# zzengcs/kubeML

Measured on AMD Instinct MI355X. Metric: images/sec (whole node) + epoch time, ResNet-34 CIFAR-10 at 1/2/4/8 workers, higher is better.
Workload: dtype bf16; 1 GPU; model=resnet34 (torchvision, ImageNet stem, 1000-class head), global_batch=256, per_worker_batch=256, image=32x32x3, parallelism=dp1, optimizer=SGD lr=0.01 wd=1e-4, sync=none (N=1: no collective in the step), graph=True, overlap_segments=False, graph_comm=False, grad_comm_dtype=fp32, sgd_rider=4f:321;123:s, step=kubeml_amd.engine.dp.make_train_step

## Files before the change

csrc/kernels/conv_igemm.hip:

```cpp
#include "kml_common.h"
#include "kml_sgd.h"

#include <type_traits>

namespace {

constexpr int PADK = 16;
constexpr int PADR = 8;

enum { FWD = 0, DGRAD = 1, WGRAD = 2 };

struct FastDiv {
  unsigned m;
  int s;
  int d;
};
__device__ __forceinline__ int fdiv(int n, const FastDiv& f) {
  return (int)(((unsigned long long)(unsigned)n * f.m) >> f.s);
}

struct ConvArgs {
  const bf16_t* x;
  const bf16_t* w;
  const bf16_t* dy;
// ... 1622 lines not shown
      return *reinterpret_cast<const bf16x8_t*>(base + (row * CPR + (c ^ (row & 15))) * 16);
    };
    f32x4_t acc[MR][NR];
#pragma unroll
    for (int i = 0; i < MR; ++i)
#pragma unroll
      for (int j = 0; j < NR; ++j) acc[i][j] = f32x4_t{0.f, 0.f, 0.f, 0.f};
    constexpr int KS = KD / 32;
    bf16x8_t af[2][MR], bf[2][NR];
#pragma unroll
    for (int i = 0; i < MR; ++i) af[0][i] = rd(sA, wm * WM + i * 16 + (lane & 15), 0);
#pragma unroll
    for (int j = 0; j < NR; ++j) bf[0][j] = rd(sB, wn * WN + j * 16 + (lane & 15), 0);
#pragma unroll
    for (int ks = 0; ks < KS; ++ks) {
      if (ks + 1 < KS) {
#pragma unroll
        for (int i = 0; i < MR; ++i) af[(ks + 1) & 1][i] = rd(sA, wm * WM + i * 16 + (lane & 15), ks + 1);
#pragma unroll
        for (int j = 0; j < NR; ++j) bf[(ks + 1) & 1][j] = rd(sB, wn * WN + j * 16 + (lane & 15), ks + 1);
      }
#pragma unroll
      for (int i = 0; i < MR; ++i)
#pragma unroll
        for (int j = 0; j < NR; ++j)
          acc[i][j] = __builtin_amdgcn_mfma_f32_16x16x32_bf16(af[ks & 1][i], bf[ks & 1][j], acc[i][j], 0, 0, 0);
    }
    __syncthreads();
    conv_epilogue<FWD, MR, NR, WM, WN, false, true>(a, acc, m0, n0, wm, wn, lane, tid, 0, 0,
                                                    reinterpret_cast<unsigned*>(smem));
  }
};

template <int MODE, int BM, int BN, int KD>
struct OneShotBwdBody {
  static_assert(MODE == DGRAD || MODE == WGRAD, "one-shot backward: dgrad / wgrad");
  static constexpr bool A_KC = MODE == DGRAD;
  static constexpr int A_BYTES = BM * KD * 2, B_BYTES = BN * KD * 2;
  static constexpr int WM = BM / 2, WN = BN / 2, MR = WM / 16, NR = WN / 16;
  static constexpr int NIA = A_BYTES / 1024, NIB = B_BYTES / 1024;
  static constexpr int SMEM_EPI = 16 + BM * (BN + 8) * 2 + 2 * BN * 4;
  static constexpr int SMEM = A_BYTES + B_BYTES > SMEM_EPI ? A_BYTES + B_BYTES : SMEM_EPI;
  static constexpr int THREADS = 256;
  static_assert(NIA % 4 == 0 && NIB % 4 == 0 && (KD / 8) % 16 == 0, "one-shot panel shape");
  static_assert((BM == 32 || BM == 64) && (BN == 32 || BN == 64), "K-strided tiles of 32 / 64 columns");
  static_assert(SMEM <= 160 * 1024, "one-shot panels exceed LDS");

  template <int R>
  __device__ __forceinline__ static void ks_slot(int L, int& k, int& lc) {
    k = L / (R / 8);
    lc = (L % (R / 8)) ^ swz_ks<R>(k);
  }

  __device__ __forceinline__ static void run(const ConvArgs& a, const Blk& bk, char* smem) {
    const int tid = threadIdx.x, lane = tid & 63, wave = tid >> 6, wm = wave >> 1, wn = wave & 1;
    const int m0 = bk.y * BM, n0 = bk.x * BN;
    const int tapoff = (a.r0 * a.KW + a.s0) * a.C;
    char* const sA = smem;
    char* const sB = smem + A_BYTES;
#pragma unroll
    for (int j = 0; j < NIA / 4; ++j) {
      const int u = j * 4 + wave, L = u * 64 + lane;
      const bf16_t* src;
      if constexpr (MODE == DGRAD) {
        const int row = L / (KD / 8), lc = (L % (KD / 8)) ^ (row & 15), m = m0 + row;
        src = m < a.M ? a.dy + (long long)m * a.K + lc * 8 : a.zp;
      } else {
        int k, lc;
        ks_slot<BM>(L, k, lc);
        const int col = m0 + lc * 8;
        src = (k < a.Kd && col < a.M) ? a.dy + (long long)k * a.K + col : a.zp;
      }
      __builtin_amdgcn_global_load_lds((const void*)src, (__attribute__((address_space(3))) void*)(sA + u * 1024),
                                       16, 0, 0);
    }
#pragma unroll
    for (int j = 0; j < NIB / 4; ++j) {
      const int u = j * 4 + wave, L = u * 64 + lane;
      int k, lc;
      ks_slot<BN>(L, k, lc);
      const int col = n0 + lc * 8;
      const bf16_t* src = a.zp;
      if constexpr (MODE == DGRAD) {
        if (k < a.K && col < a.N) {
          if (a.g22) {
            const int p = fdiv(k, a.fd_gK), q = fdiv(col, a.fd_gC);
            src = a.w + ((long long)(k - p * a.fd_gK.d) * 9 + tap22(p, q)) * a.fd_gC.d + (col - q * a.fd_gC.d);
          } else {
            src = a.w + (long long)k * a.KH * a.KW * a.C + tapoff + col;
          }
        }
      } else {
        if (k < a.Kd && col < a.N) src = a.x + (long long)k * a.C + col;
      }
      __builtin_amdgcn_global_load_lds((const void*)src, (__attribute__((address_space(3))) void*)(sB + u * 1024),
                                       16, 0, 0);
    }
    asm volatile("s_waitcnt vmcnt(0)" ::: "memory");
    __syncthreads();
    auto rdA = [&](int i, int ks) -> bf16x8_t {
      if constexpr (A_KC) {
        const int row = wm * WM + i * 16 + (lane & 15), c = 4 * ks + (lane >> 4);
        return *reinterpret_cast<const bf16x8_t*>(sA + (row * (KD / 8) + (c ^ (row & 15))) * 16);
      } else {
        return frag_kstrided<BM>(reinterpret_cast<const bf16_t*>(sA), wm * WM + i * 16, ks, lane);
      }
    };
    auto rdB = [&](int j, int ks) -> bf16x8_t {
      return frag_kstrided<BN>(reinterpret_cast<const bf16_t*>(sB), wn * WN + j * 16, ks, lane);
    };
    f32x4_t acc[MR][NR];
#pragma unroll
    for (int i = 0; i < MR; ++i)
#pragma unroll
      for (int j = 0; j < NR; ++j) acc[i][j] = f32x4_t{0.f, 0.f, 0.f, 0.f};
    constexpr int KS = KD / 32;
    bf16x8_t af[2][MR], bf[2][NR];
#pragma unroll
    for (int i = 0; i < MR; ++i) af[0][i] = rdA(i, 0);
#pragma unroll
    for (int j = 0; j < NR; ++j) bf[0][j] = rdB(j, 0);
#pragma unroll
    for (int ks = 0; ks < KS; ++ks) {
      if (ks + 1 < KS) {
#pragma unroll
        for (int i = 0; i < MR; ++i) af[(ks + 1) & 1][i] = rdA(i, ks + 1);
#pragma unroll
        for (int j = 0; j < NR; ++j) bf[(ks + 1) & 1][j] = rdB(j, ks + 1);
      }
#pragma unroll
      for (int i = 0; i < MR; ++i)
#pragma unroll
        for (int j = 0; j < NR; ++j)
          acc[i][j] = __builtin_amdgcn_mfma_f32_16x16x32_bf16(af[ks & 1][i], bf[ks & 1][j], acc[i][j], 0, 0, 0);
    }
    __syncthreads();
    conv_epilogue<MODE, MR, NR, WM, WN, false, true>(a, acc, m0, n0, wm, wn, lane, tid, 0, 0,
                                                     reinterpret_cast<unsigned*>(smem));
  }
};

template <int MODE, int BM, int BN, int KD>
__global__ __launch_bounds__(256) void k_conv_oneshot_bwd(ConvArgs a) {
  using Body = OneShotBwdBody<MODE, BM, BN, KD>;
  __shared__ __attribute__((aligned(1024))) char smem[Body::SMEM];
  Body::run(a, xcd_blk(), smem);
}

template <int MODE>
int dispatch_oneshot_bwd(const ConvArgs& a, int bm, int bn, hipStream_t s) {
  dim3 grid((a.N + bn - 1) / bn, (a.M + bm - 1) / bm, 1);
#define KML_OB(BMv, BNv, KDv)                                                              \
  if (bm == BMv && bn == BNv && a.Kd == KDv) {                                             \
    hipLaunchKernelGGL((k_conv_oneshot_bwd<MODE, BMv, BNv, KDv>), grid, dim3(256), 0, s, a); \
    KML_LAUNCH_CHECK();                                                                    \
  }
  if constexpr (MODE == DGRAD) {
    KML_OB(32, 32, 1024) KML_OB(32, 32, 512) KML_OB(32, 64, 512)
  } else {
    KML_OB(32, 32, 256) KML_OB(64, 32, 256) KML_OB(32, 64, 256) KML_OB(64, 64, 256)
  }
#undef KML_OB
  return (int)hipErrorInvalidValue;
}

template <int BM, int BN, int KD>
__global__ __launch_bounds__(256) void k_conv_oneshot(ConvArgs a) {
  using Body = OneShotBody<BM, BN, KD>;
  __shared__ __attribute__((aligned(1024))) char smem[Body::SMEM];
  Body::run(a, xcd_blk(), smem);
}
// ... 311 lines not shown
  if (id >= nd + nw) {
    kml_sgd_rider_run(rider, id - nd - nw);
    return;
  }
  if (id < nd) {
    Blk b;
    b.gx = dgx;
    b.x = id % dgx;
    const int t = id / dgx;
    b.y = t % dgy;
    b.z = t / dgy;
    DB::run(ad, b, smem);
  } else {
    id -= nd;
    Blk b;
    b.gx = wgx;
    b.x = id % wgx;
    const int t = id / wgx;
    b.y = t % wgy;
    b.z = t / wgy;
    WB::run(aw, b, smem);
  }
}

using DgIg3264 = IgemmBody<DGRAD, 32, 64, 64, true>;
using DgIg3232 = IgemmBody<DGRAD, 32, 32, 64, true>;
using DgDi3232 = DirectBody<DGRAD, 2, 2, 4, 4>;
using DgDi3216 = DirectBody<DGRAD, 2, 1, 4, 4>;
using DgDi6432 = DirectBody<DGRAD, 4, 2, 4, 2>;
using WgIg3232 = IgemmBody<WGRAD, 32, 32, 64, true>;
using WgIg6432 = IgemmBody<WGRAD, 64, 32, 64, true>;
using DgHa64x8 = HaloBody<DGRAD, 64, 8, 1, 32, 1>;
using DgHa128x4 = HaloBody<DGRAD, 128, 4, 4, 32, 1>;
#define KML_PAIR_LIST(X)                                   \
  X(4, 64, 32, 1032, DgHa64x8, 64, 32, WgIg3232, 32, 32)   \
  X(4, 64, 32, 1032, DgHa64x8, 64, 32, WgIg6432, 64, 32)   \
  X(4, 64, 32, 2052, DgHa128x4, 64, 32, WgIg3232, 32, 32)  \
  X(4, 64, 32, 2052, DgHa128x4, 64, 32, WgIg6432, 64, 32)  \
  X(0, 32, 64, 64, DgIg3264, 32, 64, WgIg3232, 32, 32)     \
  X(0, 32, 64, 64, DgIg3264, 32, 64, WgIg6432, 64, 32)     \
  X(0, 32, 32, 64, DgIg3232, 32, 32, WgIg3232, 32, 32)     \
  X(0, 32, 32, 64, DgIg3232, 32, 32, WgIg6432, 64, 32)     \
  X(3, 32, 32, 4, DgDi3232, 32, 32, WgIg3232, 32, 32)      \
  X(3, 32, 32, 4, DgDi3232, 32, 32, WgIg6432, 64, 32)      \
  X(3, 32, 16, 4, DgDi3216, 32, 16, WgIg3232, 32, 32)      \
  X(3, 32, 16, 4, DgDi3216, 32, 16, WgIg6432, 64, 32)      \
  X(3, 64, 32, 4, DgDi6432, 64, 32, WgIg3232, 32, 32)      \
  X(3, 64, 32, 4, DgDi6432, 64, 32, WgIg6432, 64, 32)

template <class DB, class WB>
int launch_pair(const ConvArgs& ad, int dbm, int dbn, const ConvArgs& aw, int wbm, int wbn, hipStream_t s) {
  const int dgx = (ad.N + dbn - 1) / dbn, dgy = (ad.M + dbm - 1) / dbm;
  const int wgx = (aw.N + wbn - 1) / wbn, wgy = (aw.M + wbm - 1) / wbm;
  const long long nd = (long long)dgx * dgy * ad.splits, nw = (long long)wgx * wgy * aw.splits;
  const KmlSgdRider rider = kml_rider_take();
  if (nd + nw + rider.blocks > 0x7fffffffLL) return (int)hipErrorInvalidValue;
  hipLaunchKernelGGL((k_conv_pair<DB, WB>), dim3((unsigned)(nd + nw + rider.blocks)), dim3(256), 0, s, ad, aw, dgx,
                     dgy, wgx, wgy, (int)nd, (int)nw, rider);
  KML_LAUNCH_CHECK();
}

int pair_index(int dv, int dbm, int dbn, int dbk, int wv, int wbm, int wbn, int wbk) {
  int idx = 0;
#define KML_PAIR_FIND(DV, DBM, DBN, DBK, DB, DTM, DTN, WB, WBM, WBN)                                   \
  ++idx;                                                                                             \
  if (dv == DV && dbm == DBM && dbn == DBN && dbk == DBK && wv == 0 && wbm == WBM && wbn == WBN && wbk == 64) \
    return idx;
  KML_PAIR_LIST(KML_PAIR_FIND)
#undef KML_PAIR_FIND
  return 0;
}

int dispatch_pair(int which, const ConvArgs& ad, const ConvArgs& aw, hipStream_t s) {
  int idx = 0;
#define KML_PAIR_RUN(DV, DBM, DBN, DBK, DB, DTM, DTN, WB, WBM, WBN) \
  if (++idx == which) return launch_pair<DB, WB>(ad, DTM, DTN, aw, WBM, WBN, s);
  KML_PAIR_LIST(KML_PAIR_RUN)
#undef KML_PAIR_RUN
  return (int)hipErrorInvalidValue;
}

template <class B1, class B2>
__global__ __launch_bounds__(256) void k_conv_fwd_pair(ConvArgs a1, ConvArgs a2, int g1x, int g1y, int g2x, int n1,
                                                       int n2) {
  static_assert(B1::THREADS == 256 && B2::THREADS == 256, "paired bodies run 256-thread blocks");
  constexpr int SM = B1::SMEM > B2::SMEM ? B1::SMEM : B2::SMEM;
  __shared__ __attribute__((aligned(1024))) char smem[SM];
  const int nwg = n1 + n2, lin = (int)blockIdx.x;
  const int q = nwg >> 3, r = nwg & 7, x = lin & 7, k = lin >> 3;
  int id = (x < r ? x * (q + 1) : r * (q + 1) + (x - r) * q) + k;
  Blk b;
  if (id < n1) {
    b.gx = g1x;
    b.x = id % g1x;
    b.y = id / g1x;
    b.z = 0;
    (void)g1y;
    B1::run(a1, b, smem);
  } else {
    id -= n1;
    b.gx = g2x;
    b.x = id % g2x;
    b.y = id / g2x;
    b.z = 0;
    B2::run(a2, b, smem);
  }
}

// ... 338 lines not shown
  set_splits(a, bk, splits);
  if (a.splits > 1 && (!slab || !counters)) return (int)hipErrorInvalidValue;
  a.slab = slab; a.counters = counters;
  a.accumulate = accumulate ? 1 : 0;
  return 0;
}
}

KML_API int kml_conv_pair_supported(int dvariant, int dbm, int dbn, int dbk, int wvariant, int wbm, int wbn, int wbk) {
  return pair_index(dvariant, dbm, dbn, dbk, wvariant, wbm, wbn, wbk) > 0 ? 1 : 0;
}

KML_API int kml_conv_bwd_pair(const bf16_t* dy, const bf16_t* w, const bf16_t* wt, bf16_t* dx, const bf16_t* addend,
                              const bf16_t* bnf_y, const bf16_t* bnf_c, const float* bnf_mean, const float* bnf_rstd,
                              float* bnf_part, float* grp_out, unsigned* grp_cnt, int grp_tiles, const bf16_t* x,
                              float* dw, int B, int H, int W, int C, int K, int KH,
                              int KW, int sh, int sw, int ph, int pw, int dbm, int dbn, int dbk, int dsplits,
                              int dvariant, float* slab, unsigned* counters, int wbm, int wbn, int wbk, int wsplits,
                              int wvariant, int fold_c, int bnf_mask_out, float* wslab, unsigned* wcounters,
                              int waccumulate, float* wbias, int wbias_acc, int g22, hipStream_t s) {
  const int which = pair_index(dvariant, dbm, dbn, dbk, wvariant, wbm, wbn, wbk);
  if (!which) return (int)hipErrorInvalidValue;
  if (dvariant == 4 && (g22 || fold_c || dsplits != 1 || dbk != K * 16 + H ||
                        !halo_shape_ok(H, W, K, C, KH, KW, sh, sw, ph, pw, dbm, dbn)))
    return (int)hipErrorInvalidValue;
  ConvArgs ad, aw;
  int e = prep_dgrad(ad, dy, w, wt, dx, addend, bnf_y, bnf_c, bnf_mean, bnf_rstd, bnf_part, grp_out, grp_cnt,
                     grp_tiles, B, H, W, C, K, KH, KW, sh, sw, ph, pw, dbk, dsplits, dvariant, slab, counters,
                     fold_c, bnf_mask_out, g22);
  if (e) return e;
  e = prep_wgrad(aw, x, dy, dw, B, H, W, C, K, KH, KW, sh, sw, ph, pw, wbk, wsplits, wvariant, waccumulate, wslab,
                 wcounters, wbias, wbias_acc);
  if (e) return e;
  return dispatch_pair(which, ad, aw, s);
}

KML_API int kml_weight_transpose_multi(const bf16_t* const* ws, bf16_t* const* wts, const int* dims, int n,
                                       hipStream_t s) {
  if (n < 1 || n > 16) return (int)hipErrorInvalidValue;
  TransposeBatch tb = {};
  tb.n = n;
  long long tiles = 0;
  for (int i = 0; i < n; ++i) {
    TransposeJob& j = tb.j[i];
    j.w = ws[i]; j.wt = wts[i];
    j.K = dims[4 * i]; j.T = dims[4 * i + 1]; j.C = dims[4 * i + 2];
    if (j.C % 8) return (int)hipErrorInvalidValue;
    j.Kp = (j.K + 31) / 32 * 32;
    j.tk = (j.Kp + 63) / 64;
    j.tc = (j.C + 63) / 64;
    j.tile_begin = (int)tiles;
    tiles += (long long)j.T * j.tk * j.tc;
  }
  if (tiles <= 0 || tiles > 0x7fffffffLL) return (int)hipErrorInvalidValue;
  hipLaunchKernelGGL(k_weight_transpose_multi, dim3((unsigned)tiles), dim3(256), 0, s, tb);
  KML_LAUNCH_CHECK();
}

KML_API int kml_conv_unroll22_multi(const bf16_t* const* ws, bf16_t* const* wus, const int* dims, int n,
                                    hipStream_t s) {
  if (n < 1 || n > 16) return (int)hipErrorInvalidValue;
  UnrollBatch ub = {};
  ub.n = n;
  long long blocks = 0;
  for (int i = 0; i < n; ++i) {
    UnrollJob& j = ub.j[i];
// ... 194 lines not shown
```

kubeml_amd/nn/fused.py:

```python
from __future__ import annotations

from typing import List, Optional

import torch
from torch.autograd import Function

import os

from .flat import grad_out, grad_out_pair, master_of, shadow_of

_BN_FUSE = True


def _wg_buf(conv, x):
    Kc, _, _, C = conv.weight._kml_grad_storage.shape
    shape = (4 * Kc, 1, 1, 4 * C)
    buf = getattr(conv, "_kml_wg_buf", None)
    if buf is None or tuple(buf.shape) != shape or buf.device != x.device:
        buf = torch.empty(shape, dtype=torch.float32, device=x.device)
        object.__setattr__(conv, "_kml_wg_buf", buf)
    return buf


def _wgrad_target(conv, x, unroll):
# ... 187 lines not shown
        c = K.conv_fwd(x, w, kh, kw, conv.stride, conv.padding, bias=bias)
        y = K.bn_apply(c, None, gamma, beta, res=res, run_mean=bn.running_mean, run_var=bn.running_var,
                       eps=bn.eps, relu=relu, training=False)
        return y, None

    @staticmethod
    def backward(dy, saved, conv, bn, want_dres: bool, need_dx: bool, addend=None, partial=None, consumer=None):
        dc, dres, wu = ConvBNUnit.bn_backward(dy, saved, conv, bn, want_dres, partial)
        dx, part_out = ConvBNUnit.conv_backward(dc, saved, conv, need_dx, wu, addend, consumer)
        return dx, dres, part_out

    @staticmethod
    def bn_backward(dy, saved, conv, bn, want_dres: bool, partial=None):
        from ..ops import kernels as K
        x, c, y, mean, rstd = saved
        dg, db, acc = grad_out_pair(bn.weight, bn.bias)
        wu = getattr(conv, "_kml_wu", None) if x.is_cuda else None
        dres = torch.empty_like(dy) if want_dres else None
        dc = K.bn_bwd(dy, None if partial is not None else y, c, mean, rstd, master_of(bn.weight),
                      dg, db, dres=dres, partial=partial, accumulate=acc, rider=_take_rider(bn))
        object.__setattr__(conv, "_kml_wu", None)
        return dc, dres, wu

    @staticmethod
    def conv_backward(dc, saved, conv, need_dx: bool, wu, addend=None, consumer=None):
        from ..ops import kernels as K
        x = saved[0]
        kh, kw = conv.kernel_size
        dx, part_out = None, None
        bnf = None if consumer is None else (consumer[2], consumer[1], consumer[3], consumer[4])
        if need_dx:
            w = shadow_of(conv.weight)
            wt = getattr(conv, "_kml_wt", None)
            if wt is None and K.bwd_plans(x.shape, w.shape[0], kh, kw, conv.stride, conv.padding,
                                          unroll=wu is not None)[0][4] == K.DIRECT:
                object.__setattr__(conv, "_kml_wants_wt", True)
            dw, acc = _wgrad_target(conv, x, wu is not None)
            r = K.conv_bwd(dc, w, x, dw, kh, kw, conv.stride, conv.padding,
                           addend=addend, bnf=bnf, wt=wt, wu=wu, bnf_mask=True, accumulate=acc,
                           rider=_take_rider(conv))
            if wu is not None:
                conv.weight._kml_flat.defer_fold22(conv.weight, dw)
            object.__setattr__(conv, "_kml_wt", None)
            dx, part_out = r if bnf is not None else (r, None)
            return dx, part_out
        _wgrad(x, dc, conv, unroll=wu is not None, rider=_take_rider(conv))
        if need_dx:
            r = K.conv_dgrad(dc, shadow_of(conv.weight), x.shape, kh, kw, conv.stride, conv.padding,
                             addend=addend, bnf=bnf, wu=wu, bnf_mask=True)
            dx, part_out = r if bnf is not None else (r, None)
        return dx, part_out


def _take_rider(conv):
    r = getattr(conv, "_kml_rider", None)
    return r() if r is not None else None


class PendingBN:
    __slots__ = ("y", "c", "rows", "G", "bn", "res", "mean", "rstd", "relu")

    def __init__(self, y, c, rows, G, bn, res, mean, rstd, relu):
        self.y, self.c, self.rows, self.G, self.bn = y, c, rows, G, bn
        self.res, self.mean, self.rstd, self.relu = res, mean, rstd, relu

    def materialize(self):
        from ..ops import kernels as K
        bn = self.bn
        K.bn_apply(self.c, self.rows, master_of(bn.weight), master_of(bn.bias), y=self.y, res=self.res,
                   save_mean=self.mean, save_rstd=self.rstd, run_mean=bn.running_mean, run_var=bn.running_var,
                   eps=bn.eps, momentum=bn.momentum if bn.momentum is not None else 0.1, relu=self.relu,
                   stats_rows=self.G)


# ... 233 lines not shown
```

kubeml_amd/ops/kernels.py:

```python
from __future__ import annotations

import contextlib
import json
import math
import os

import torch

from .. import _native
from .._native import HIP

BF16 = torch.bfloat16
F32 = torch.float32


def _s() -> int:
    return _native.stream_ptr()


def _p(t) -> int:
    return 0 if t is None else t.data_ptr()


def _chk(t, dtype, name, ndim=None):
# ... 432 lines not shown
def gemm_dgrad_gather_ok(C, K, stride) -> bool:
    return tuple(stride) == (1, 1) and K % 64 == 0 and C % 8 == 0


def gemm_conv_ok(C, K, H, W, KH, KW, stride, pad) -> bool:
    return C % 64 == 0 and K % 8 == 0


def oneshot_ok(C, K, Kd, H, W, KH, KW, stride, pad, bm, bn) -> bool:
    if Kd != C or (bm, bn) not in _ONESHOT_TILES.get(Kd, ()):
        return False
    r0, r1, s0, s1 = tap_window(H, W, KH, KW, stride[0], stride[1], pad[0], pad[1])
    OH, OW = out_hw(H, W, KH, KW, stride[0], stride[1], pad[0], pad[1])
    rows = (H * W == 1 and OH * OW == 1) or ((KH, KW) == (1, 1) and tuple(stride) == (1, 1) and tuple(pad) == (0, 0))
    return (r1 - r0) == 1 and (s1 - s0) == 1 and rows


_ONESHOT_MAX_ROWS = 4096


def oneshot_plan(C, K, Kd, H, W, KH, KW, stride, pad, B=0):
    if B * H * W > _ONESHOT_MAX_ROWS:
        return None
    for bm, bn in _ONESHOT_TILES.get(Kd, ()):
        if oneshot_ok(C, K, Kd, H, W, KH, KW, stride, pad, bm, bn):
            return (bm, bn, 0, 1, ONESHOT)
    return None


_ONESHOT_BWD_ON = False
_ONESHOT_DG_TILES = {1024: (32, 32), 512: (32, 32)}
_ONESHOT_WG_TILES = {256: (32, 32)}


def oneshot_bwd_plans(C, K, B, H, W, KH, KW, stride, pad):
    if not _ONESHOT_BWD_ON or C % 32 or K % 32:
        return None, None
    r0, r1, s0, s1 = tap_window(H, W, KH, KW, stride[0], stride[1], pad[0], pad[1])
    OH, OW = out_hw(H, W, KH, KW, stride[0], stride[1], pad[0], pad[1])
    rows = (H * W == 1 and OH * OW == 1) or ((KH, KW) == (1, 1) and tuple(stride) == (1, 1) and tuple(pad) == (0, 0))
    if not ((r1 - r0) == 1 and (s1 - s0) == 1 and rows):
        return None, None
    d = _ONESHOT_DG_TILES.get(K)
    w = _ONESHOT_WG_TILES.get(B * OH * OW)
    return ((d[0], d[1], 0, 1, ONESHOT) if d else None), ((w[0], w[1], 0, 1, ONESHOT) if w else None)


def halo_plan(C, K, H, W, KH, KW, stride, pad):
    for bm, bn in _HALO_TILES.get((C, H), ()):
        if halo_ok(C, K, H, W, KH, KW, stride, pad, bm, bn):
            return (bm, bn, 0, 1, HALO)
    return None


def conv_fwd_stats_rows(x_shape, K, KH, KW, stride, pad, cfg=None, unroll=False, group=False):
    B, H, W, C = x_shape
    if unroll:
        if not unrolled22(H, W, KH, KW, stride, pad):
            raise ValueError("conv is not unrolled")
        return 4 * conv_stats_rows(B, conv_fwd_plan(4 * C, B, 4 * K, 4 * C, cfg, geom=(1, 1, 1, 1, (1, 1), (0, 0))))
    OH, OW = out_hw(H, W, KH, KW, stride[0], stride[1], pad[0], pad[1])
    r0, r1, s0, s1 = tap_window(H, W, KH, KW, stride[0], stride[1], pad[0], pad[1])
    M, Kd = B * OH * OW, (r1 - r0) * (s1 - s0) * C
    return conv_stats_rows(M, conv_fwd_plan(C, M, K, Kd, cfg, geom=(H, W, KH, KW, stride, pad)), group)


# ... 225 lines not shown
def _bnf_ws(bnf, out, M, C, plan, fold=0):
    if bnf is None:
        return None, None, None, None, None, None, None, None, 0, 0
    by, bc, bmean, brstd = bnf
    if bc.shape != out.shape or (by is not None and by.shape != out.shape):
        raise ValueError("bnf tensors must match the dgrad output shape")
    G = conv_stats_rows(M, plan)
    part = torch.empty(G * 2 * C, dtype=F32, device=out.device)
    rows, grp, gcnt, tpg = _stats_ws(out.device, M, C, plan, part)
    if fold:
        if grp is not None or C % fold:
            raise ValueError("folded BN partials cannot be group-reduced")
        G *= C // fold
    return by, bc, bmean, brstd, part, rows, grp, gcnt, tpg, G


def _direct_wt(w, wt):
    K, KH, KW, C = w.shape
    Kp = _cdiv(K, 32) * 32
    if wt is None:
        wt = torch.empty((C, KH, KW, Kp), dtype=BF16, device=w.device)
        HIP.call("kml_weight_transpose", "p p i i i i s", _p(w), _p(wt), K, KH, KW, C, _s())
    elif tuple(wt.shape) != (C, KH, KW, Kp) or wt.dtype != BF16:
        raise ValueError("transposed weight shape mismatch")
    return wt


def dgrad_plan(in_shape, K, KH, KW, stride, pad, cfg=None):
    B, H, W, C = in_shape
    r0, r1, s0, s1 = tap_window(H, W, KH, KW, stride[0], stride[1], pad[0], pad[1])
    return _norm_cfg(cfg or plan_conv("dgrad", B * H * W, C, (r1 - r0) * (s1 - s0) * K))


def bwd_plans(in_shape, K, KH, KW, stride, pad, dcfg=None, wcfg=None, unroll=False):
    B, H, W, C = in_shape
    if unroll:
        return bwd_plans((B, 1, 1, 4 * C), 4 * K, 1, 1, (1, 1), (0, 0), dcfg, wcfg)
    sh, sw = stride
    ph, pw = pad
    OH, OW = out_hw(H, W, KH, KW, sh, sw, ph, pw)
    r0, r1, s0, s1 = tap_window(H, W, KH, KW, sh, sw, ph, pw)
    ntap = (r1 - r0) * (s1 - s0)
    if dcfg is None and wcfg is None:
        dcfg, wcfg = _TUNED_PAIR.get((B * H * W, C, ntap * K, K, ntap * C, B * OH * OW), (None, None))
        hp = halo_dgrad_plan(C, K, H, W, KH, KW, stride, pad)
        if hp is not None:
            dcfg = hp
        od, ow = oneshot_bwd_plans(C, K, B, H, W, KH, KW, stride, pad)
        dcfg, wcfg = od or dcfg, ow or wcfg
    dplan = _norm_cfg(dcfg or plan_conv("dgrad", B * H * W, C, ntap * K))
    wplan = _norm_cfg(wcfg or plan_conv("wgrad", K, ntap * C, B * OH * OW))
    return dplan, wplan, conv_pair_supported(dplan, wplan)


_PAIR_OK: dict = {}


def conv_pair_supported(dcfg, wcfg) -> bool:
    key = (tuple(dcfg), tuple(wcfg))
    ok = _PAIR_OK.get(key)
    if ok is None:
        dbm, dbn, dbk, _, dv = dcfg
        wbm, wbn, wbk, _, wv = wcfg
        ok = _PAIR_OK[key] = bool(HIP.fn("kml_conv_pair_supported", "i i i i i i i i")(
            dv, dbm, dbn, dbk, wv, wbm, wbn, wbk))
    return ok


def conv_bwd(dy, w, x, dw, KH, KW, stride, pad, addend=None, bnf=None, wt=None, dcfg=None, wcfg=None, wu=None,
             bnf_mask=False, accumulate=True, dbias=None, bias_accumulate=True, rider=None):
    _chk(dy, BF16, "dy", 4)
    _chk(w, BF16, "w", 4)
    _chk(x, BF16, "x", 4)
    _chk(dw, F32, "dw", 4)
    B, H, W, C = x.shape
    K = w.shape[0]
    sh, sw = stride
    ph, pw = pad
    OH, OW = out_hw(H, W, KH, KW, sh, sw, ph, pw)
    want_dw = (4 * K, 1, 1, 4 * C) if wu is not None else (K, KH, KW, C)
    if tuple(dy.shape) != (B, OH, OW, K) or tuple(w.shape) != (K, KH, KW, C) or tuple(dw.shape) != want_dw:
        raise ValueError("conv_bwd shape mismatch")
    if K % 8 or C % 8:
        raise ValueError("channels must be multiples of 8")
    fold, g22 = 0, False
    if wu is not None:
        _check_wu(x.shape, w, wu, KH, KW, stride, pad)
        dy, x, addend, bnf = _u22_views(B, C, K, dy=dy, x=x, addend=addend, bnf=bnf)
        g22 = wu is GATHER22
        w, fold, accumulate = (w if g22 else wu), C, False
        H = W = OH = OW = 1
        KH = KW = sh = sw = 1
        ph = pw = 0
        C, K = 4 * C, 4 * K
        stride, pad = (1, 1), (0, 0)
    r0, r1, s0, s1 = tap_window(H, W, KH, KW, sh, sw, ph, pw)
    ntap = (r1 - r0) * (s1 - s0)
    M = B * H * W
    dplan, wplan, grouped = bwd_plans(x.shape, K, KH, KW, stride, pad, dcfg, wcfg)
    wroute = None if (wcfg is not None or wu is not None) else wgrad_gemm_route(x.shape, K, KH, KW, stride, pad, dbias)
    if wroute is not None:
        grouped = False
    if grouped and s2_parity_ok(B, H, W, stride, dplan, g22, fold, operands=addend is not None or bnf is not None):
        grouped = False
    if dbias is not None and wu is not None:
        raise ValueError("conv_bwd: dbias needs a 1x1 conv")
    if not grouped:
        conv_wgrad(x, dy, dw, KH, KW, stride, pad, cfg=None if wroute is not None else wplan, accumulate=accumulate,
                   dbias=dbias, bias_accumulate=bias_accumulate)
        r = conv_dgrad(dy, w, (B, H, W, C), KH, KW, stride, pad, addend=addend, cfg=dplan, bnf=bnf, wt=wt, _fold=fold,
                       bnf_mask=bnf_mask, _g22=g22)
        if rider is not None:
            rider.run_alone()
        if not fold:
            return r
        if bnf is not None:
            return r[0].view(B, 2, 2, C // 4), r[1]
        return r.view(B, 2, 2, C // 4)
    bm, bn, bk, splits, variant = dplan
    out = torch.empty((B, H, W, C), dtype=BF16, device=dy.device)
    if addend is not None:
        _chk(addend, BF16, "addend")
        assert addend.shape == out.shape
    by, bc, bmean, brstd, part, rows, grp, gcnt, tpg, G = _bnf_ws(bnf, out, M, C, dplan, fold)
    slab = cnt = None
    if variant in (HALO, ONESHOT):
        wt, dsplits = None, 1
    elif variant == DIRECT:
        if g22:
            raise ValueError("the direct dgrad variant needs a materialised unrolled weight (not GATHER22)")
        wt = _direct_wt(w, wt)
        dsplits = 1
    else:
        wt = None
        dsplits = effective_splits(ntap * _cdiv(K, bk) * bk, bk, splits)
        slab, cnt = _splitk_ws(dy.device, M, C, bm, bn, dsplits)
    wbm, wbn, wbk, wsplits, wvariant = wplan
    _chk_dbias(dbias, K, KH, KW, stride, pad)
    wslab, wcnt = _wgrad_ws(dw.device, B, H, W, C, K, KH, KW, stride, pad, wplan, dbias is not None)
    with _Riding(rider):
        HIP.call("kml_conv_bwd_pair",
                 "p p p p p p p p p p p p i p p i i i i i i i i i i i i i i i i p p i i i i i i i p p i p i i s",
                 _p(dy), _p(w), _p(wt), _p(out), _p(addend), _p(by), _p(bc), _p(bmean), _p(brstd), _p(rows),
                 _p(grp), _p(gcnt), tpg, _p(x), _p(dw), B, H, W, C, K, KH, KW, sh, sw, ph, pw, bm, bn, bk, dsplits,
                 variant, _p(slab), _p(cnt), wbm, wbn, wbk, wsplits, wvariant, int(fold),
                 int(bool(bnf_mask) and bnf is not None), _p(wslab), _p(wcnt), int(bool(accumulate)), _p(dbias),
                 int(bool(bias_accumulate)), int(g22), _s())
    if fold:
        out = out.view(B, 2, 2, C // 4)
    return (out, (part, G)) if bnf is not None else out


def weight_transpose_multi(ws, wts):
    import ctypes
    n = len(ws)
    if n == 0:
        return
    if n > 16 or len(wts) != n:
        raise ValueError("weight_transpose_multi: 1..16 pairs")
    wp = (ctypes.c_void_p * n)()
    tp = (ctypes.c_void_p * n)()
    dims = (ctypes.c_int * (4 * n))()
    for i, (w, wt) in enumerate(zip(ws, wts)):
        _chk(w, BF16, "w", 4)
        _chk(wt, BF16, "wt", 4)
        K, KH, KW, C = w.shape
        if tuple(wt.shape) != (C, KH, KW, _cdiv(K, 32) * 32):
            raise ValueError("transposed weight shape mismatch")
        wp[i], tp[i] = w.data_ptr(), wt.data_ptr()
        dims[4 * i], dims[4 * i + 1], dims[4 * i + 2] = K, KH * KW, C
    HIP.call("kml_weight_transpose_multi", "p p p i s", ctypes.addressof(wp), ctypes.addressof(tp),
             ctypes.addressof(dims), n, _s())
# ... 610 lines not shown
```

Measured before the change: 198,300 images/s.

## Add one-shot dgrad/wgrad pair with folded 2x2 wgrad for small-pixel convs

Adds paired one-shot backward variants: the dgrad body can load K in two passes to fit LDS, and a new wgrad body computes the unrolled 2x2 conv gradient and folds it straight into the (K,3,3,C) weight layout. The planner sends small-pixel 1x1/1x1-spatial convs to these pairs, skipping split-K workspaces and the deferred fold22 pass. This cuts launches and scratch traffic for the deep ResNet layers, at the cost of more template variants and stricter shape preconditions. Dispatch falls back when the preconditions fail.

```diff
diff --git a/csrc/kernels/conv_igemm.hip b/csrc/kernels/conv_igemm.hip
--- a/csrc/kernels/conv_igemm.hip
+++ b/csrc/kernels/conv_igemm.hip
@@ -1678,17 +1678,19 @@
   }
 };
 
-template <int MODE, int BM, int BN, int KD>
+template <int MODE, int BM, int BN, int KD, int NH = 1>
 struct OneShotBwdBody {
   static_assert(MODE == DGRAD || MODE == WGRAD, "one-shot backward: dgrad / wgrad");
+  static_assert(NH == 1 || MODE == DGRAD, "K in passes: dgrad only");
   static constexpr bool A_KC = MODE == DGRAD;
-  static constexpr int A_BYTES = BM * KD * 2, B_BYTES = BN * KD * 2;
+  static constexpr int KP = KD / NH;
+  static constexpr int A_BYTES = BM * KP * 2, B_BYTES = BN * KP * 2;
   static constexpr int WM = BM / 2, WN = BN / 2, MR = WM / 16, NR = WN / 16;
   static constexpr int NIA = A_BYTES / 1024, NIB = B_BYTES / 1024;
   static constexpr int SMEM_EPI = 16 + BM * (BN + 8) * 2 + 2 * BN * 4;
   static constexpr int SMEM = A_BYTES + B_BYTES > SMEM_EPI ? A_BYTES + B_BYTES : SMEM_EPI;
   static constexpr int THREADS = 256;
-  static_assert(NIA % 4 == 0 && NIB % 4 == 0 && (KD / 8) % 16 == 0, "one-shot panel shape");
+  static_assert(KD % NH == 0 && NIA % 4 == 0 && NIB % 4 == 0 && (KP / 8) % 16 == 0, "one-shot panel shape");
   static_assert((BM == 32 || BM == 64) && (BN == 32 || BN == 64), "K-strided tiles of 32 / 64 columns");
   static_assert(SMEM <= 160 * 1024, "one-shot panels exceed LDS");
 
@@ -1704,50 +1706,10 @@
     const int tapoff = (a.r0 * a.KW + a.s0) * a.C;
     char* const sA = smem;
     char* const sB = smem + A_BYTES;
-#pragma unroll
-    for (int j = 0; j < NIA / 4; ++j) {
-      const int u = j * 4 + wave, L = u * 64 + lane;
-      const bf16_t* src;
-      if constexpr (MODE == DGRAD) {
-        const int row = L / (KD / 8), lc = (L % (KD / 8)) ^ (row & 15), m = m0 + row;
-        src = m < a.M ? a.dy + (long long)m * a.K + lc * 8 : a.zp;
-      } else {
-        int k, lc;
-        ks_slot<BM>(L, k, lc);
-        const int col = m0 + lc * 8;
-        src = (k < a.Kd && col < a.M) ? a.dy + (long long)k * a.K + col : a.zp;
-      }
-      __builtin_amdgcn_global_load_lds((const void*)src, (__attribute__((address_space(3))) void*)(sA + u * 1024),
-                                       16, 0, 0);
-    }
-#pragma unroll
-    for (int j = 0; j < NIB / 4; ++j) {
-      const int u = j * 4 + wave, L = u * 64 + lane;
-      int k, lc;
-      ks_slot<BN>(L, k, lc);
-      const int col = n0 + lc * 8;
-      const bf16_t* src = a.zp;
-      if constexpr (MODE == DGRAD) {
-        if (k < a.K && col < a.N) {
-          if (a.g22) {
-            const int p = fdiv(k, a.fd_gK), q = fdiv(col, a.fd_gC);
-            src = a.w + ((long long)(k - p * a.fd_gK.d) * 9 + tap22(p, q)) * a.fd_gC.d + (col - q * a.fd_gC.d);
-          } else {
-            src = a.w + (long long)k * a.KH * a.KW * a.C + tapoff + col;
-          }
-        }
-      } else {
-        if (k < a.Kd && col < a.N) src = a.x + (long long)k * a.C + col;
-      }
-      __builtin_amdgcn_global_load_lds((const void*)src, (__attribute__((address_space(3))) void*)(sB + u * 1024),
-                                       16, 0, 0);
-    }
-    asm volatile("s_waitcnt vmcnt(0)" ::: "memory");
-    __syncthreads();
     auto rdA = [&](int i, int ks) -> bf16x8_t {
       if constexpr (A_KC) {
         const int row = wm * WM + i * 16 + (lane & 15), c = 4 * ks + (lane >> 4);
-        return *reinterpret_cast<const bf16x8_t*>(sA + (row * (KD / 8) + (c ^ (row & 15))) * 16);
+        return *reinterpret_cast<const bf16x8_t*>(sA + (row * (KP / 8) + (c ^ (row & 15))) * 16);
       } else {
         return frag_kstrided<BM>(reinterpret_cast<const bf16_t*>(sA), wm * WM + i * 16, ks, lane);
       }
@@ -1760,29 +1722,166 @@
     for (int i = 0; i < MR; ++i)
 #pragma unroll
       for (int j = 0; j < NR; ++j) acc[i][j] = f32x4_t{0.f, 0.f, 0.f, 0.f};
-    constexpr int KS = KD / 32;
-    bf16x8_t af[2][MR], bf[2][NR];
-#pragma unroll
-    for (int i = 0; i < MR; ++i) af[0][i] = rdA(i, 0);
-#pragma unroll
-    for (int j = 0; j < NR; ++j) bf[0][j] = rdB(j, 0);
-#pragma unroll
-    for (int ks = 0; ks < KS; ++ks) {
-      if (ks + 1 < KS) {
-#pragma unroll
-        for (int i = 0; i < MR; ++i) af[(ks + 1) & 1][i] = rdA(i, ks + 1);
-#pragma unroll
-        for (int j = 0; j < NR; ++j) bf[(ks + 1) & 1][j] = rdB(j, ks + 1);
+#pragma unroll
+    for (int h = 0; h < NH; ++h) {
+      const int kh = h * KP;
+      if (h) __syncthreads();
+#pragma unroll
+      for (int j = 0; j < NIA / 4; ++j) {
+        const int u = j * 4 + wave, L = u * 64 + lane;
+        const bf16_t* src;
+        if constexpr (MODE == DGRAD) {
+          const int row = L / (KP / 8), lc = (L % (KP / 8)) ^ (row & 15), m = m0 + row;
+          src = m < a.M ? a.dy + (long long)m * a.K + kh + lc * 8 : a.zp;
+        } else {
+          int k, lc;
+          ks_slot<BM>(L, k, lc);
+          const int col = m0 + lc * 8;
+          src = (k < a.Kd && col < a.M) ? a.dy + (long long)k * a.K + col : a.zp;
+        }
+        __builtin_amdgcn_global_load_lds((const void*)src, (__attribute__((address_space(3))) void*)(sA + u * 1024),
+                                         16, 0, 0);
       }
 #pragma unroll
-      for (int i = 0; i < MR; ++i)
-#pragma unroll
-        for (int j = 0; j < NR; ++j)
-          acc[i][j] = __builtin_amdgcn_mfma_f32_16x16x32_bf16(af[ks & 1][i], bf[ks & 1][j], acc[i][j], 0, 0, 0);
+      for (int j = 0; j < NIB / 4; ++j) {
+        const int u = j * 4 + wave, L = u * 64 + lane;
+        int k, lc;
+        ks_slot<BN>(L, k, lc);
+        const int col = n0 + lc * 8;
+        const bf16_t* src = a.zp;
+        if constexpr (MODE == DGRAD) {
+          k += kh;
+          if (k < a.K && col < a.N) {
+            if (a.g22) {
+              const int p = fdiv(k, a.fd_gK), q = fdiv(col, a.fd_gC);
+              src = a.w + ((long long)(k - p * a.fd_gK.d) * 9 + tap22(p, q)) * a.fd_gC.d + (col - q * a.fd_gC.d);
+            } else {
+              src = a.w + (long long)k * a.KH * a.KW * a.C + tapoff + col;
+            }
+          }
+        } else {
+          if (k < a.Kd && col < a.N) src = a.x + (long long)k * a.C + col;
+        }
+        __builtin_amdgcn_global_load_lds((const void*)src, (__attribute__((address_space(3))) void*)(sB + u * 1024),
+                                         16, 0, 0);
+      }
+      asm volatile("s_waitcnt vmcnt(0)" ::: "memory");
+      __syncthreads();
+      constexpr int KS = KP / 32;
+      bf16x8_t af[2][MR], bf[2][NR];
+#pragma unroll
+      for (int i = 0; i < MR; ++i) af[0][i] = rdA(i, 0);
+#pragma unroll
+      for (int j = 0; j < NR; ++j) bf[0][j] = rdB(j, 0);
+#pragma unroll
+      for (int ks = 0; ks < KS; ++ks) {
+        if (ks + 1 < KS) {
+#pragma unroll
+          for (int i = 0; i < MR; ++i) af[(ks + 1) & 1][i] = rdA(i, ks + 1);
+#pragma unroll
+          for (int j = 0; j < NR; ++j) bf[(ks + 1) & 1][j] = rdB(j, ks + 1);
+        }
+#pragma unroll
+        for (int i = 0; i < MR; ++i)
+#pragma unroll
+          for (int j = 0; j < NR; ++j)
+            acc[i][j] = __builtin_amdgcn_mfma_f32_16x16x32_bf16(af[ks & 1][i], bf[ks & 1][j], acc[i][j], 0, 0, 0);
+      }
     }
     __syncthreads();
     conv_epilogue<MODE, MR, NR, WM, WN, false, true>(a, acc, m0, n0, wm, wn, lane, tid, 0, 0,
                                                      reinterpret_cast<unsigned*>(smem));
+  }
+};
+
+template <int KD>
+struct OneShotFold22Body {
+  static constexpr int TK = 16, TC = 16, R = 64;
+  static constexpr int P_BYTES = KD * R * 2;
+  static constexpr int NI = P_BYTES / 1024;
+  static constexpr int SMEM = 2 * P_BYTES;
+  static constexpr int THREADS = 256;
+  static_assert(NI % 4 == 0 && KD % 32 == 0, "folded one-shot panel shape");
+
+  __device__ __forceinline__ static void run(const ConvArgs& a, const Blk& bk, char* smem) {
+    const int tid = threadIdx.x, lane = tid & 63, wave = __builtin_amdgcn_readfirstlane(tid >> 6);
+    const int k0 = bk.y * TK, c0 = bk.x * TC;
+    const int Kq = a.fd_gK.d, Cq = a.fd_gC.d;
+    char* const sA = smem;
+    char* const sB = smem + P_BYTES;
+    const unsigned pairs = wave == 0 ? 0x0F0A0500u : wave == 1 ? 0x07020D08u : wave == 2 ? 0x0B010E04u : 0x0306090Cu;
+    int pp[4], qq[4];
+#pragma unroll
+    for (int t = 0; t < 4; ++t) {
+      pp[t] = (pairs >> (8 * t + 2)) & 3;
+      qq[t] = (pairs >> (8 * t)) & 3;
+    }
+    f32x4_t acc[4];
+#pragma unroll
+    for (int t = 0; t < 4; ++t) acc[t] = f32x4_t{0.f, 0.f, 0.f, 0.f};
+#pragma unroll
+    for (int j = 0; j < NI / 4; ++j) {
+      const int u = j * 4 + wave, L = u * 64 + lane;
+      const int k = L / (R / 8), lc = (L % (R / 8)) ^ swz_ks<R>(k);
+      const int pos = lc >> 1, off = (lc & 1) * 8;
+      const bf16_t* sa = (k < a.Kd && k0 + off < Kq) ? a.dy + (long long)k * a.K + pos * Kq + k0 + off : a.zp;
+      const bf16_t* sb = (k < a.Kd && c0 + off < Cq) ? a.x + (long long)k * a.C + pos * Cq + c0 + off : a.zp;
+      __builtin_amdgcn_global_load_lds((const void*)sa, (__attribute__((address_space(3))) void*)(sA + u * 1024),
+                                       16, 0, 0);
+      __builtin_amdgcn_global_load_lds((const void*)sb, (__attribute__((address_space(3))) void*)(sB + u * 1024),
+                                       16, 0, 0);
+    }
+    asm volatile("s_waitcnt vmcnt(0)" ::: "memory");
+    __syncthreads();
+    constexpr int KS = KD / 32;
+    bf16x8_t af[2][4], bf[2][4];
+#pragma unroll
+    for (int t = 0; t < 4; ++t) {
+      af[0][t] = frag_kstrided<R>(reinterpret_cast<const bf16_t*>(sA), pp[t] * 16, 0, lane);
+      bf[0][t] = frag_kstrided<R>(reinterpret_cast<const bf16_t*>(sB), qq[t] * 16, 0, lane);
+    }
+#pragma unroll
+    for (int ks = 0; ks < KS; ++ks) {
+      if (ks + 1 < KS) {
+#pragma unroll
+        for (int t = 0; t < 4; ++t) {
+          af[(ks + 1) & 1][t] = frag_kstrided<R>(reinterpret_cast<const bf16_t*>(sA), pp[t] * 16, ks + 1, lane);
+          bf[(ks + 1) & 1][t] = frag_kstrided<R>(reinterpret_cast<const bf16_t*>(sB), qq[t] * 16, ks + 1, lane);
+        }
+      }
+#pragma unroll
+      for (int t = 0; t < 4; ++t)
+        acc[t] = __builtin_amdgcn_mfma_f32_16x16x32_bf16(af[ks & 1][t], bf[ks & 1][t], acc[t], 0, 0, 0);
+    }
+    unsigned heads = 0xFu;
+    if (wave == 0) {
+#pragma unroll
+      for (int e = 0; e < 4; ++e) acc[0][e] = ((acc[0][e] + acc[1][e]) + acc[2][e]) + acc[3][e];
+      heads = 0x1u;
+    } else if (wave != 3) {
+#pragma unroll
+      for (int e = 0; e < 4; ++e) {
+        acc[0][e] += acc[1][e];
+        acc[2][e] += acc[3][e];
+      }
+      heads = 0x5u;
+    }
+    const int fr = lane & 15, fq = lane >> 4;
+    const int col = c0 + fr;
+#pragma unroll
+    for (int t = 0; t < 4; ++t) {
+      if (!((heads >> t) & 1u) || col >= Cq) continue;
+      const int tap = tap22(pp[t], qq[t]);
+#pragma unroll
+      for (int e = 0; e < 4; ++e) {
+        const int row = k0 + fq * 4 + e;
+        if (row < Kq) {
+          float* p = a.dw + ((long long)row * 9 + tap) * Cq + col;
+          if (a.accumulate) *p += acc[t][e];
+          else *p = acc[t][e];
+        }
+      }
+    }
   }
 };
 
@@ -2160,21 +2259,30 @@
 using WgIg6432 = IgemmBody<WGRAD, 64, 32, 64, true>;
 using DgHa64x8 = HaloBody<DGRAD, 64, 8, 1, 32, 1>;
 using DgHa128x4 = HaloBody<DGRAD, 128, 4, 4, 32, 1>;
-#define KML_PAIR_LIST(X)                                   \
-  X(4, 64, 32, 1032, DgHa64x8, 64, 32, WgIg3232, 32, 32)   \
-  X(4, 64, 32, 1032, DgHa64x8, 64, 32, WgIg6432, 64, 32)   \
-  X(4, 64, 32, 2052, DgHa128x4, 64, 32, WgIg3232, 32, 32)  \
-  X(4, 64, 32, 2052, DgHa128x4, 64, 32, WgIg6432, 64, 32)  \
-  X(0, 32, 64, 64, DgIg3264, 32, 64, WgIg3232, 32, 32)     \
-  X(0, 32, 64, 64, DgIg3264, 32, 64, WgIg6432, 64, 32)     \
-  X(0, 32, 32, 64, DgIg3232, 32, 32, WgIg3232, 32, 32)     \
-  X(0, 32, 32, 64, DgIg3232, 32, 32, WgIg6432, 64, 32)     \
-  X(3, 32, 32, 4, DgDi3232, 32, 32, WgIg3232, 32, 32)      \
-  X(3, 32, 32, 4, DgDi3232, 32, 32, WgIg6432, 64, 32)      \
-  X(3, 32, 16, 4, DgDi3216, 32, 16, WgIg3232, 32, 32)      \
-  X(3, 32, 16, 4, DgDi3216, 32, 16, WgIg6432, 64, 32)      \
-  X(3, 64, 32, 4, DgDi6432, 64, 32, WgIg3232, 32, 32)      \
-  X(3, 64, 32, 4, DgDi6432, 64, 32, WgIg6432, 64, 32)
+using DgOs1024 = OneShotBwdBody<DGRAD, 32, 32, 1024>;
+using DgOs1024h = OneShotBwdBody<DGRAD, 32, 32, 1024, 2>;
+using DgOs512 = OneShotBwdBody<DGRAD, 32, 32, 512>;
+using WgOs256 = OneShotBwdBody<WGRAD, 32, 32, 256>;
+using WgFo256 = OneShotFold22Body<256>;
+constexpr int WV_FOLD22 = 8;
+#define KML_PAIR_LIST(X)                                          \
+  X(4, 64, 32, 1032, DgHa64x8, 64, 32, WgIg3232, 32, 32, 0, 64)   \
+  X(4, 64, 32, 1032, DgHa64x8, 64, 32, WgIg6432, 64, 32, 0, 64)   \
+  X(4, 64, 32, 2052, DgHa128x4, 64, 32, WgIg3232, 32, 32, 0, 64)  \
+  X(4, 64, 32, 2052, DgHa128x4, 64, 32, WgIg6432, 64, 32, 0, 64)  \
+  X(0, 32, 64, 64, DgIg3264, 32, 64, WgIg3232, 32, 32, 0, 64)     \
+  X(0, 32, 64, 64, DgIg3264, 32, 64, WgIg6432, 64, 32, 0, 64)     \
+  X(0, 32, 32, 64, DgIg3232, 32, 32, WgIg3232, 32, 32, 0, 64)     \
+  X(0, 32, 32, 64, DgIg3232, 32, 32, WgIg6432, 64, 32, 0, 64)     \
+  X(3, 32, 32, 4, DgDi3232, 32, 32, WgIg3232, 32, 32, 0, 64)      \
+  X(3, 32, 32, 4, DgDi3232, 32, 32, WgIg6432, 64, 32, 0, 64)      \
+  X(3, 32, 16, 4, DgDi3216, 32, 16, WgIg3232, 32, 32, 0, 64)      \
+  X(3, 32, 16, 4, DgDi3216, 32, 16, WgIg6432, 64, 32, 0, 64)      \
+  X(3, 64, 32, 4, DgDi6432, 64, 32, WgIg3232, 32, 32, 0, 64)      \
+  X(3, 64, 32, 4, DgDi6432, 64, 32, WgIg6432, 64, 32, 0, 64)      \
+  X(5, 32, 32, 1024, DgOs1024, 32, 32, WgFo256, 16, 16, 8, 256)   \
+  X(5, 32, 32, 1025, DgOs1024h, 32, 32, WgFo256, 16, 16, 8, 256)  \
+  X(5, 32, 32, 512, DgOs512, 32, 32, WgOs256, 32, 32, 5, 256)
 
 template <class DB, class WB>
 int launch_pair(const ConvArgs& ad, int dbm, int dbn, const ConvArgs& aw, int wbm, int wbn, hipStream_t s) {
@@ -2190,9 +2298,9 @@
 
 int pair_index(int dv, int dbm, int dbn, int dbk, int wv, int wbm, int wbn, int wbk) {
   int idx = 0;
-#define KML_PAIR_FIND(DV, DBM, DBN, DBK, DB, DTM, DTN, WB, WBM, WBN)                                   \
-  ++idx;                                                                                             \
-  if (dv == DV && dbm == DBM && dbn == DBN && dbk == DBK && wv == 0 && wbm == WBM && wbn == WBN && wbk == 64) \
+#define KML_PAIR_FIND(DV, DBM, DBN, DBK, DB, DTM, DTN, WB, WBM, WBN, WV, WBK)                            \
+  ++idx;                                                                                              \
+  if (dv == DV && dbm == DBM && dbn == DBN && dbk == DBK && wv == WV && wbm == WBM && wbn == WBN && wbk == WBK) \
     return idx;
   KML_PAIR_LIST(KML_PAIR_FIND)
 #undef KML_PAIR_FIND
@@ -2201,7 +2309,7 @@
 
 int dispatch_pair(int which, const ConvArgs& ad, const ConvArgs& aw, hipStream_t s) {
   int idx = 0;
-#define KML_PAIR_RUN(DV, DBM, DBN, DBK, DB, DTM, DTN, WB, WBM, WBN) \
+#define KML_PAIR_RUN(DV, DBM, DBN, DBK, DB, DTM, DTN, WB, WBM, WBN, WV, WBK) \
   if (++idx == which) return launch_pair<DB, WB>(ad, DTM, DTN, aw, WBM, WBN, s);
   KML_PAIR_LIST(KML_PAIR_RUN)
 #undef KML_PAIR_RUN
@@ -2606,6 +2714,20 @@
   e = prep_wgrad(aw, x, dy, dw, B, H, W, C, K, KH, KW, sh, sw, ph, pw, wbk, wsplits, wvariant, waccumulate, wslab,
                  wcounters, wbias, wbias_acc);
   if (e) return e;
+  const bool one_tap = (ad.r1 - ad.r0) == 1 && (ad.s1 - ad.s0) == 1;
+  const bool rows = (H * W == 1 && ad.OH * ad.OW == 1) || (KH == 1 && KW == 1 && sh == 1 && sw == 1 && !ph && !pw);
+  if (dvariant == 5) {
+    if (!one_tap || !rows || ad.splits != 1 || (dbk & ~1) != K) return (int)hipErrorInvalidValue;
+    ad.Kd = K;
+  }
+  if (wvariant == 5 || wvariant == WV_FOLD22) {
+    if (!one_tap || !rows || wbias || aw.splits != 1 || aw.Kd > wbk) return (int)hipErrorInvalidValue;
+  }
+  if (wvariant == WV_FOLD22) {
+    if (H * W != 1 || KH != 1 || KW != 1 || K % 32 || C % 32) return (int)hipErrorInvalidValue;
+    aw.fd_gK = make_fd(K / 4); aw.fd_gC = make_fd(C / 4);
+    aw.M = K / 4; aw.N = C / 4;
+  }
   return dispatch_pair(which, ad, aw, s);
 }
 
diff --git a/kubeml_amd/nn/fused.py b/kubeml_amd/nn/fused.py
--- a/kubeml_amd/nn/fused.py
+++ b/kubeml_amd/nn/fused.py
@@ -243,14 +243,16 @@
         if need_dx:
             w = shadow_of(conv.weight)
             wt = getattr(conv, "_kml_wt", None)
-            if wt is None and K.bwd_plans(x.shape, w.shape[0], kh, kw, conv.stride, conv.padding,
-                                          unroll=wu is not None)[0][4] == K.DIRECT:
+            dplan, wplan, _ = K.bwd_plans(x.shape, w.shape[0], kh, kw, conv.stride, conv.padding,
+                                          unroll=wu is not None)
+            if wt is None and dplan[4] == K.DIRECT:
                 object.__setattr__(conv, "_kml_wants_wt", True)
-            dw, acc = _wgrad_target(conv, x, wu is not None)
+            folded = wu is not None and wplan[4] == K.FOLD22
+            dw, acc = _wgrad_target(conv, x, wu is not None and not folded)
             r = K.conv_bwd(dc, w, x, dw, kh, kw, conv.stride, conv.padding,
                            addend=addend, bnf=bnf, wt=wt, wu=wu, bnf_mask=True, accumulate=acc,
                            rider=_take_rider(conv))
-            if wu is not None:
+            if wu is not None and not folded:
                 conv.weight._kml_flat.defer_fold22(conv.weight, dw)
             object.__setattr__(conv, "_kml_wt", None)
             dx, part_out = r if bnf is not None else (r, None)
diff --git a/kubeml_amd/ops/kernels.py b/kubeml_amd/ops/kernels.py
--- a/kubeml_amd/ops/kernels.py
+++ b/kubeml_amd/ops/kernels.py
@@ -488,6 +488,30 @@
 _ONESHOT_DG_TILES = {1024: (32, 32), 512: (32, 32)}
 _ONESHOT_WG_TILES = {256: (32, 32)}
 
+_ONESHOT_PAIR_ON = True
+_ONESHOT_PAIR_PIXELS = 256
+FOLD22 = 8
+_ONESHOT_PAIR_U22_FULL = ((32, 32, 1024, 1, ONESHOT), (16, 16, 256, 1, FOLD22))
+_ONESHOT_PAIR_U22_HALF = ((32, 32, 1025, 1, ONESHOT), (16, 16, 256, 1, FOLD22))
+_ONESHOT_PAIR_U22 = _ONESHOT_PAIR_U22_HALF
+
+
+def oneshot_pair_plans(C, K, B, H, W, KH, KW, stride, pad, fold22=False):
+    if not _ONESHOT_PAIR_ON or _ONESHOT_BWD_ON or C % 32 or K % 32:
+        return None, None
+    r0, r1, s0, s1 = tap_window(H, W, KH, KW, stride[0], stride[1], pad[0], pad[1])
+    OH, OW = out_hw(H, W, KH, KW, stride[0], stride[1], pad[0], pad[1])
+    rows = (H * W == 1 and OH * OW == 1) or ((KH, KW) == (1, 1) and tuple(stride) == (1, 1) and tuple(pad) == (0, 0))
+    if not ((r1 - r0) == 1 and (s1 - s0) == 1 and rows) or B * OH * OW > _ONESHOT_PAIR_PIXELS:
+        return None, None
+    if fold22:
+        d, w = _ONESHOT_PAIR_U22
+        if (d[2] & ~1) != K or H * W != 1:
+            return None, None
+    else:
+        d, w = (32, 32, K, 1, ONESHOT), (32, 32, _ONESHOT_PAIR_PIXELS, 1, ONESHOT)
+    return (d, w) if conv_pair_supported(d, w) else (None, None)
+
 
 def oneshot_bwd_plans(C, K, B, H, W, KH, KW, stride, pad):
     if not _ONESHOT_BWD_ON or C % 32 or K % 32:
@@ -779,15 +803,24 @@
     return _norm_cfg(cfg or plan_conv("dgrad", B * H * W, C, (r1 - r0) * (s1 - s0) * K))
 
 
-def bwd_plans(in_shape, K, KH, KW, stride, pad, dcfg=None, wcfg=None, unroll=False):
+def bwd_plans(in_shape, K, KH, KW, stride, pad, dcfg=None, wcfg=None, unroll=False, scratch=False,
+              oneshot_pair=True):
     B, H, W, C = in_shape
     if unroll:
-        return bwd_plans((B, 1, 1, 4 * C), 4 * K, 1, 1, (1, 1), (0, 0), dcfg, wcfg)
+        if dcfg is None and wcfg is None and not scratch and oneshot_pair:
+            od, ow = oneshot_pair_plans(4 * C, 4 * K, B, 1, 1, 1, 1, (1, 1), (0, 0), fold22=True)
+            if od is not None:
+                return od, ow, True
+        return bwd_plans((B, 1, 1, 4 * C), 4 * K, 1, 1, (1, 1), (0, 0), dcfg, wcfg, oneshot_pair=False)
     sh, sw = stride
     ph, pw = pad
     OH, OW = out_hw(H, W, KH, KW, sh, sw, ph, pw)
     r0, r1, s0, s1 = tap_window(H, W, KH, KW, sh, sw, ph, pw)
     ntap = (r1 - r0) * (s1 - s0)
+    if dcfg is None and wcfg is None and oneshot_pair:
+        od, ow = oneshot_pair_plans(C, K, B, H, W, KH, KW, stride, pad)
+        if od is not None:
+            return od, ow, True
     if dcfg is None and wcfg is None:
         dcfg, wcfg = _TUNED_PAIR.get((B * H * W, C, ntap * K, K, ntap * C, B * OH * OW), (None, None))
         hp = halo_dgrad_plan(C, K, H, W, KH, KW, stride, pad)
@@ -825,7 +858,8 @@
     sh, sw = stride
     ph, pw = pad
     OH, OW = out_hw(H, W, KH, KW, sh, sw, ph, pw)
-    want_dw = (4 * K, 1, 1, 4 * C) if wu is not None else (K, KH, KW, C)
+    folded = wu is not None and tuple(dw.shape) == (K, KH, KW, C)
+    want_dw = (4 * K, 1, 1, 4 * C) if (wu is not None and not folded) else (K, KH, KW, C)
     if tuple(dy.shape) != (B, OH, OW, K) or tuple(w.shape) != (K, KH, KW, C) or tuple(dw.shape) != want_dw:
         raise ValueError("conv_bwd shape mismatch")
     if K % 8 or C % 8:
@@ -833,9 +867,18 @@
     fold, g22 = 0, False
     if wu is not None:
         _check_wu(x.shape, w, wu, KH, KW, stride, pad)
+        if folded:
+            if dcfg is not None or wcfg is not None:
+                raise ValueError("conv_bwd: the folded route (a (K,3,3,C) dw with wu) runs its own plans")
+            dcfg, wcfg, ok = bwd_plans(x.shape, K, KH, KW, stride, pad, unroll=True)
+            if not ok or wcfg[4] != FOLD22:
+                raise ValueError("conv_bwd: no folded one-shot pair for this unrolled conv "
+                                 "(pass the [4K,1,1,4C] scratch as dw and fold with fold22_multi)")
         dy, x, addend, bnf = _u22_views(B, C, K, dy=dy, x=x, addend=addend, bnf=bnf)
         g22 = wu is GATHER22
-        w, fold, accumulate = (w if g22 else wu), C, False
+        w, fold = (w if g22 else wu), C
+        if not folded:
+            accumulate = False
         H = W = OH = OW = 1
         KH = KW = sh = sw = 1
         ph = pw = 0
@@ -844,8 +887,13 @@
     r0, r1, s0, s1 = tap_window(H, W, KH, KW, sh, sw, ph, pw)
     ntap = (r1 - r0) * (s1 - s0)
     M = B * H * W
-    dplan, wplan, grouped = bwd_plans(x.shape, K, KH, KW, stride, pad, dcfg, wcfg)
-    wroute = None if (wcfg is not None or wu is not None) else wgrad_gemm_route(x.shape, K, KH, KW, stride, pad, dbias)
+    if folded:
+        dplan, wplan, grouped = dcfg, wcfg, True
+    else:
+        dplan, wplan, grouped = bwd_plans(x.shape, K, KH, KW, stride, pad, dcfg, wcfg,
+                                          oneshot_pair=dbias is None and wu is None)
+    wroute = None if (wcfg is not None or wu is not None or wplan[4] == ONESHOT) else \
+        wgrad_gemm_route(x.shape, K, KH, KW, stride, pad, dbias)
     if wroute is not None:
         grouped = False
     if grouped and s2_parity_ok(B, H, W, stride, dplan, g22, fold, operands=addend is not None or bnf is not None):
@@ -884,7 +932,10 @@
         slab, cnt = _splitk_ws(dy.device, M, C, bm, bn, dsplits)
     wbm, wbn, wbk, wsplits, wvariant = wplan
     _chk_dbias(dbias, K, KH, KW, stride, pad)
-    wslab, wcnt = _wgrad_ws(dw.device, B, H, W, C, K, KH, KW, stride, pad, wplan, dbias is not None)
+    if wplan[4] in (ONESHOT, FOLD22):
+        wslab = wcnt = None
+    else:
+        wslab, wcnt = _wgrad_ws(dw.device, B, H, W, C, K, KH, KW, stride, pad, wplan, dbias is not None)
     with _Riding(rider):
         HIP.call("kml_conv_bwd_pair",
                  "p p p p p p p p p p p p i p p i i i i i i i i i i i i i i i i p p i i i i i i i p p i p i i s",
```

After: 207,100 images/s, median of 6. 4.4% higher.
